# patflick/psac

Hardware: AMD Instinct MI355X
Metric: MChars/s SA+LCP build; rank-pair radix-sort HBM GB/s vs peak (higher is better)
Workload: dtype u64

## Files before the change

psac_amd/csrc/engine.hpp:

```cpp
#pragma once
#include <hip/hip_runtime.h>

#include <algorithm>
#include <cstdio>
#include <cstdlib>
#include <cstring>
#include <condition_variable>
#include <functional>
#include <map>
#include <mutex>
#include <string>
#include <thread>
#include <sched.h>
#include <pthread.h>
#include <cctype>
#include <cstdio>
#include <vector>

#include "../../include/psacx.h"
#include "radix.hpp"
#include "sa_kernels.hpp"

namespace psacx {

// ... 802 lines not shown
        } else {
            ProfScope ps(c, TC_SORT_SCATTER);
            if (small_desc) dispatch_scatter<T, uint32_t>(c, kd_in, ko_in, v_in, kd_out, ko_out, v_out, n, plan.shift[p], base, desc, sc.d_err, spec, spec_n);
            else dispatch_scatter<T, uint64_t>(c, kd_in, ko_in, v_in, kd_out, ko_out, v_out, n, plan.shift[p], base, desc, sc.d_err, spec, spec_n);
            PSACX_HIP(c, hipGetLastError());
        }
        const int form = !in.k2 ? 2 : (three ? 1 : 0);
        c->stats.scatter_launches[form] += 1;
        c->stats.scatter_records[form] += n;
        if (narrow) c->stats.scatter_bytes[form] += ((in.k2 ? 4ull : 2ull) * sizeof(T) + (v_in ? ((first && !v32_in) ? sizeof(T) : 4ull) : 0ull) + (last ? sizeof(T) : 4ull) + (dig_next ? 1ull : 0ull)) * n;
        else c->stats.scatter_bytes[form] += ((in.k2 ? 6ull : 4ull) - (v_in ? 0ull : 1ull)) * sizeof(T) * n;
        std::swap(cur, oth);
        cur.v = v_out;
    }
    if (n_exec == 0) {
        T* dst = final_v ? final_v : cur.v;
        if (iota) {
            hipLaunchKernelGGL((iota_kernel<T>), dim3(grid_for(c, n, 256)), dim3(256), 0, c->stream, dst, n, spec, spec_n);
            PSACX_HIP(c, hipGetLastError());
        } else if (v32_in && keep_v32) {
            dst = cur.v;
        } else if (v32_in) {
            T* const w = (dst == cur.v) ? oth.v : dst;
            hipLaunchKernelGGL((widen32_kernel<T>), dim3(grid_for(c, n, 256)), dim3(256), 0, c->stream, reinterpret_cast<const uint32_t*>(cur.v), n, w);
            PSACX_HIP(c, hipGetLastError());
            if (w != dst) PSACX_HIP(c, hipMemcpyAsync(dst, w, n * sizeof(T), hipMemcpyDeviceToDevice, c->stream));
        } else if (dst != cur.v) {
            PSACX_HIP(c, hipMemcpyAsync(dst, cur.v, n * sizeof(T), hipMemcpyDeviceToDevice, c->stream));
        }
        cur.v = dst;
    }
    *res = cur;
    return PSACX_OK;
}

constexpr int PSACX_RETRY_1W = 1001;
constexpr int PSACX_RETRY_1STAGE = 1002;
#ifndef PSACX_1W_ITEMS
#define PSACX_1W_ITEMS 8
#endif
inline int onew_bucket_passes(psacx_ctx* c, char* scratch, const unsigned long long* h_tabs, const OneWordLayout& lay, uint64_t* cur, uint64_t* oth, uint64_t* sa_out,
                              unsigned sfield, unsigned low, unsigned lo1, uint64_t nrec, uint64_t** s1, OneWordView* view_out = nullptr, uint8_t* dig = nullptr,
                              uint64_t in_pad = 0, uint8_t* tie_bytes = nullptr, unsigned long long* h_word = nullptr, bool* tie_bits = nullptr) {
    constexpr int BLOCK = 512, ITEMS_B = PSACX_1W_ITEMS, TILE = BLOCK * ITEMS_B;
    unsigned* tile_hist = reinterpret_cast<unsigned*>(scratch + lay.tile_hist);
    unsigned long long* slab_tot = reinterpret_cast<unsigned long long*>(scratch + lay.slab_tot);
    unsigned long long* base2 = reinterpret_cast<unsigned long long*>(scratch + lay.base2);
    unsigned long long* d_tabs = reinterpret_cast<unsigned long long*>(scratch + lay.tabs);
    OneWordTabs tb;
    tb.bucket_off = d_tabs; tb.slab_start = d_tabs + RADIX + 1; tb.slab = lay.slab;
    SlabInfo* slab_info = reinterpret_cast<SlabInfo*>(scratch + lay.slab_info);
    tb.slab_info = slab_info;
    *s1 = cur;
    if (tie_bits) *tie_bits = false;
    if (view_out) { view_out->off = d_tabs; view_out->low = low; view_out->sfield = sfield; view_out->lo1 = lo1; }
    PSACX_HIP(c, hipMemcpyAsync(d_tabs, h_tabs, 2 * (RADIX + 1) * sizeof(unsigned long long), hipMemcpyHostToDevice, c->stream));
    if (lay.total_slabs == 0) return PSACX_OK;
    const uint64_t total_slabs = lay.total_slabs, vtiles = lay.vtiles;
    hipLaunchKernelGGL(radix_slab_info_kernel<0>, dim3((unsigned)((total_slabs + 255) / 256)), dim3(256), 0, c->stream, tb.bucket_off, tb.slab_start,
                       (unsigned)total_slabs, (unsigned)(lay.slab * TILE), slab_info);
    PSACX_HIP(c, hipGetLastError());
    const int npass = (int)((low + RADIX_BITS - 1) / RADIX_BITS);
    bool first = true;
    auto tables = [&](const OneWordTabs& t, int shift, bool from_bytes, unsigned long long* dbase) {
        ProfScope ps(c, TC_SORT_TILEHIST);
        const uint64_t nt = t.tile_sub ? lay.sub_tiles : vtiles;
        if (from_bytes) hipLaunchKernelGGL((radix_tile_hist_bytes_kernel<BLOCK, ITEMS_B>), dim3((unsigned)((nt + BLOCK / WAVE - 1) / (BLOCK / WAVE))), dim3(BLOCK), 0, c->stream,
                                           (const uint8_t*)dig, t, (unsigned)nt, tile_hist);
        else
        hipLaunchKernelGGL((radix_tile_hist1w_kernel<BLOCK, ITEMS_B>), dim3((unsigned)nt), dim3(BLOCK), 0, c->stream, (const uint64_t*)cur, t, shift, tile_hist,
                           first ? in_pad : (uint64_t)0);
        if (t.tile_sub) hipLaunchKernelGGL(radix_sub_scan1w_kernel<0>, dim3(ONEW_SUB), dim3(RADIX), 0, c->stream, tile_hist, t, dbase);
        else {
            hipLaunchKernelGGL(radix_slab_scan1w_kernel<0>, dim3((unsigned)total_slabs), dim3(RADIX), 0, c->stream, tile_hist, t, (unsigned)TILE, slab_tot);
            hipLaunchKernelGGL(radix_top_scan1w_kernel<0>, dim3(RADIX), dim3(RADIX), 0, c->stream, slab_tot, t, dbase);
        }
    };
    auto scatter = [&](const OneWordTabs& t, int shift, bool widen, const unsigned long long* dbase, uint8_t* dnext, int dnext_shift) -> int {
        ProfScope ps(c, TC_SORT_SCATTER2);
        const uint64_t nt = t.tile_sub ? lay.sub_tiles : vtiles;
        PSACX_HIP(c, hipMemsetAsync(scratch, 0, 256, c->stream));
        if (!widen)
            hipLaunchKernelGGL((radix_scatter1w_kernel<BLOCK, ITEMS_B, 8>), dim3((unsigned)nt), dim3(BLOCK), 0, c->stream, (const uint64_t*)cur, oth, (uint64_t*)nullptr, shift,
                               t, dbase, tile_hist, slab_tot, reinterpret_cast<unsigned*>(scratch), sort_chunk_for(nrec, true), 0u,
                               dnext, dnext_shift, first ? in_pad : (uint64_t)0);
        else
            hipLaunchKernelGGL((radix_scatter1w_kernel<BLOCK, ITEMS_B, 9>), dim3((unsigned)nt), dim3(BLOCK), 0, c->stream, (const uint64_t*)cur, oth, sa_out, shift,
                               t, dbase, tile_hist, slab_tot, reinterpret_cast<unsigned*>(scratch), sort_chunk_for(nrec, true), lo1 | (low << 8) | (sfield << 16),
                               (uint8_t*)nullptr, 0, first ? in_pad : (uint64_t)0);
        PSACX_HIP(c, hipGetLastError());
        c->stats.scatter_launches[2] += 1; c->stats.scatter_records[2] += nrec; c->stats.scatter_bytes[2] += ((widen ? 24ull : 16ull) + (dnext ? 1ull : 0ull)) * nrec;
        c->stats.onew_passes += 1;
        std::swap(cur, oth);
        first = false;
        return PSACX_OK;
    };
    auto lsd = [&](const OneWordTabs& t, int nd, unsigned long long* dbase) -> int {
        for (int j = 0; j < nd; ++j) {
            const bool last = j + 1 == nd, widen = last && !view_out;
            const int shift = (int)sfield + j * RADIX_BITS;
            tables(t, shift, dig && j > 0, dbase);
            PSACX_HIP(c, hipGetLastError());
            PSACX_TRY(scatter(t, shift, widen, dbase, widen ? (uint8_t*)nullptr : last ? tie_bytes : dig, last ? (int)sfield : shift + RADIX_BITS));
        }
        return PSACX_OK;
    };
    if (!(lay.group && view_out && dig && tie_bytes && h_word)) {
        PSACX_TRY(lsd(tb, npass, base2));
        *s1 = cur;
        return PSACX_OK;
    }
    unsigned long long* const max_word = reinterpret_cast<unsigned long long*>(scratch + lay.max_word);
    const int mid_shift = (int)sfield + 2 * RADIX_BITS;
    OneWordTabs tg = tb;
    unsigned long long* gbase = base2;
    uint64_t ngroups = (uint64_t)RADIX * RADIX;
    if (low == 32) {
        unsigned long long* const sub_off = reinterpret_cast<unsigned long long*>(scratch + lay.sub_off);
        unsigned long long* const zero_row = reinterpret_cast<unsigned long long*>(scratch + lay.zero_row);
        unsigned* const first_tile = reinterpret_cast<unsigned*>(scratch + lay.first_tile);
        unsigned* const tile_sub = reinterpret_cast<unsigned*>(scratch + lay.tile_sub);
        tables(tb, mid_shift + RADIX_BITS, false, sub_off);
        PSACX_HIP(c, hipGetLastError());
        PSACX_TRY(scatter(tb, mid_shift + RADIX_BITS, false, sub_off, dig, mid_shift));
        {
            ProfScope ps(c, TC_SORT_TILEHIST);
            PSACX_HIP(c, hipMemcpyAsync(sub_off + ONEW_SUB, h_tabs + RADIX, sizeof(unsigned long long), hipMemcpyHostToDevice, c->stream));
            PSACX_HIP(c, hipMemsetAsync(zero_row, 0, (size_t)RADIX * 8, c->stream));
            PSACX_HIP(c, hipMemsetAsync(tile_sub, 0xFF, (size_t)lay.sub_tiles * 4, c->stream));
            hipLaunchKernelGGL(onew_sub_first_tile_kernel<1024>, dim3(1), dim3(1024), 0, c->stream, sub_off, ONEW_SUB, (unsigned)TILE, first_tile);
            hipLaunchKernelGGL(onew_sub_tile_fill_kernel<256>, dim3(ONEW_SUB / (256 / WAVE)), dim3(256), 0, c->stream, first_tile, ONEW_SUB, (unsigned)lay.sub_tiles, tile_sub);
            PSACX_HIP(c, hipGetLastError());
        }
        tg.bucket_off = sub_off; tg.tile_sub = tile_sub; tg.first_tile = first_tile; tg.zero_row = zero_row;
        gbase = reinterpret_cast<unsigned long long*>(scratch + lay.group_base);
        ngroups = (uint64_t)ONEW_SUB * RADIX;
        tables(tg, mid_shift, true, gbase);
    } else
        tables(tb, mid_shift, false, gbase);
    PSACX_HIP(c, hipMemsetAsync(max_word, 0, 16, c->stream));
    hipLaunchKernelGGL(onew_max_group_kernel<256>, dim3((unsigned)grid_for(c, ngroups, 256, 8)), dim3(256), 0, c->stream, gbase, ngroups, nrec, max_word);
    PSACX_HIP(c, hipGetLastError());
    PSACX_HIP(c, hipMemcpyAsync(h_word, max_word, sizeof(unsigned long long), hipMemcpyDeviceToHost, c->stream));
    PSACX_HIP(c, hipStreamSynchronize(c->stream));
    if (*h_word > (unsigned long long)GROUP_CAP) {
        c->stats.group_sort = 2;
        PSACX_TRY(lsd(tg, 3, gbase));
        *s1 = cur;
        return PSACX_OK;
    }
    PSACX_TRY(scatter(tg, mid_shift, false, gbase, (uint8_t*)nullptr, 0));
    {
        ProfScope ps(c, TC_SORT_SCATTER2);
        const dim3 grid((unsigned)grid_for(c, ngroups, 256, 5));
        const bool bits = tie_bits && !c->knobs.plain_side_kernels && !c->knobs.tie_bytes;
        if (bits) PSACX_HIP(c, hipMemsetAsync(tie_bytes, 0, (size_t)((nrec + 63) / 64) * 8, c->stream));
        if (bits && c->knobs.group_counting_rounds)
            hipLaunchKernelGGL((group_sort16_kernel<256, false, true>), grid, dim3(256), 0, c->stream, cur, gbase, ngroups, nrec, (int)sfield, tie_bytes);
        else if (bits)
            hipLaunchKernelGGL((group_sort16_kernel<256, true, true>), grid, dim3(256), 0, c->stream, cur, gbase, ngroups, nrec, (int)sfield, tie_bytes);
        else if (c->knobs.group_counting_rounds)
            hipLaunchKernelGGL((group_sort16_kernel<256, false>), grid, dim3(256), 0, c->stream, cur, gbase, ngroups, nrec, (int)sfield, tie_bytes);
        else
            hipLaunchKernelGGL((group_sort16_kernel<256, true>), grid, dim3(256), 0, c->stream, cur, gbase, ngroups, nrec, (int)sfield, tie_bytes);
        PSACX_HIP(c, hipGetLastError());
        if (bits) *tie_bits = true;
        c->stats.scatter_launches[2] += 1; c->stats.scatter_records[2] += nrec; c->stats.scatter_bytes[2] += 17ull * nrec;
        c->stats.onew_passes += 1;
    }
    c->stats.group_sort = 1;
    *s1 = cur;
    return PSACX_OK;
}
inline int prefix_sort_1w(psacx_ctx* c, SortScratch& sc, uint64_t* k0, uint64_t* a, uint64_t* sa_out, uint64_t n, unsigned lo1, unsigned lead,
                          psacx_round* rs, uint64_t** s1, const uint8_t* text, uint64_t n_text, const CodeTable& tab, const KeyShape& ks, bool probe,
                          OneWordView* view_out = nullptr, uint8_t* dig = nullptr, uint64_t pad = 0, uint8_t* tie_bytes = nullptr, bool* tie_bits = nullptr) {
    constexpr int BLOCK = 512, ITEMS = 8, TILE0 = BLOCK * ITEMS;
    constexpr int TILE = BLOCK * PSACX_1W_ITEMS;
    const unsigned low = lead - RADIX_BITS;
    const unsigned sfield = 64 - low;
    const uint64_t ntiles = (n + TILE0 - 1) / TILE0;
    char* const scratch = sc.d_desc;
    const PassScratch p0 = pass_scratch(scratch, ntiles);
    unsigned long long* base0 = sc.d_base;
    {
        ProfScope ps(c, TC_KMER);
        const uint64_t stride = std::max<uint64_t>(64, n >> 20), samples = n / stride;
        uint64_t slots = 1; while (slots < 4 * samples) slots <<= 1;
        unsigned long long* table = reinterpret_cast<unsigned long long*>(scratch + 256);
        unsigned long long* d_dups = reinterpret_cast<unsigned long long*>(scratch + 128);
        if (256 + slots * 8 <= sc.desc_bytes && samples >= 1024 && probe) {
            PSACX_HIP(c, hipMemsetAsync(scratch, 0, 256 + slots * 8, c->stream));
            hipLaunchKernelGGL((prefix_dup_probe_kernel<uint64_t>), dim3((unsigned)((samples + 255) / 256)), dim3(256), 0, c->stream, text, n_text, tab, ks, lo1,
                               stride, samples, table, slots, d_dups);
            PSACX_HIP(c, hipGetLastError());
            PSACX_HIP(c, hipMemcpyAsync(sc.h_base, d_dups, sizeof(unsigned long long), hipMemcpyDeviceToHost, c->stream));
            PSACX_HIP(c, hipStreamSynchronize(c->stream));
            if (sc.h_base[0] * 4 >= samples * 3) return PSACX_RETRY_1STAGE;
            if (sc.h_base[0] * 8 > samples) return PSACX_RETRY_1W;
        }
        static_assert(TILE0 == 64 * WAVE, "top_digit_hist_waves_kernel: a wave takes a tile of 64 records per lane");
        if (c->knobs.plain_side_kernels || (reinterpret_cast<uintptr_t>(p0.tile_hist) & 15u))
            hipLaunchKernelGGL((top_digit_hist_kernel<uint64_t, BLOCK, ITEMS>), dim3((unsigned)ntiles), dim3(BLOCK), 0, c->stream, text, n, n_text, tab, ks, p0.tile_hist);
        else
            hipLaunchKernelGGL((top_digit_hist_waves_kernel<256>), dim3((unsigned)grid_for(c, ntiles * WAVE, 256, 5)), dim3(256), 0, c->stream, text, n, n_text, tab, ks,
                               ntiles, p0.tile_hist);
        PSACX_HIP(c, hipGetLastError());
    }
    {
        ProfScope ps(c, TC_SORT_TILEHIST);
        launch_pass_scans(c, p0, base0);
        PSACX_HIP(c, hipGetLastError());
    }
    PSACX_HIP(c, hipMemcpyAsync(sc.h_base, base0, RADIX * sizeof(unsigned long long), hipMemcpyDeviceToHost, c->stream));
    PSACX_HIP(c, hipStreamSynchronize(c->stream));
    unsigned long long* h_tabs = sc.h_base + (PIN_TABS - PIN_BASE) / sizeof(unsigned long long);
    for (int d = 0; d < RADIX; ++d) h_tabs[d] = sc.h_base[d];
    h_tabs[RADIX] = n;
    OneWordLayout lay = onew_layout<TILE>(h_tabs, ntiles);
    if (lay.need > sc.desc_bytes || lay.vtiles >= (1ull << 31)) return PSACX_RETRY_1W;
    if (view_out && dig && tie_bytes && !c->knobs.lsd_bucket_passes) lay = onew_group_layout<TILE>(lay, n, low, sc.desc_bytes);
    unsigned long long* const h_word = sc.h_base + (PIN_GROUP_WORD - PIN_BASE) / sizeof(unsigned long long);
    {
        ProfScope ps(c, TC_KMER);
        PSACX_HIP(c, hipMemsetAsync(scratch, 0, 256, c->stream));
        hipLaunchKernelGGL((key_scatter1w_kernel<BLOCK, ITEMS>), dim3((unsigned)ntiles), dim3(BLOCK), 0, c->stream, text, n, n_text, tab, ks, pad ? k0 : a, (int)(lo1 + low),
                           base0, p0.tile_hist, p0.slab_tot, p0.counter, sort_chunk_for(n, true), p0.slab_tiles, lo1 | (sfield << 16), (uint64_t)0,
                           (uint8_t*)nullptr, 0, pad);
        PSACX_HIP(c, hipGetLastError());
    }
    uint64_t* cur = nullptr;
    if (pad) PSACX_TRY(onew_bucket_passes(c, scratch, h_tabs, lay, k0, a, sa_out, sfield, low, lo1, n, &cur, view_out, dig, pad, tie_bytes, h_word, tie_bits));
    else PSACX_TRY(onew_bucket_passes(c, scratch, h_tabs, lay, a, k0, sa_out, sfield, low, lo1, n, &cur, view_out, dig, 0, tie_bytes, h_word, tie_bits));
    *s1 = cur;
    if (rs) { rs->sort_passes = (uint32_t)((low + RADIX_BITS - 1) / RADIX_BITS + 1); rs->sort_passes_skipped = 0; }
    return PSACX_OK;
}

}
```

psac_amd/csrc/radix.hpp:

```cpp
#pragma once
#include <type_traits>
#include "dev_common.hpp"
#include "sort_scratch.hpp"
#include "group_rank.hpp"
#include "tie_bits.hpp"

namespace psacx {


struct PassPlan {
    int n_pass;
    int word[MAX_PASSES];
    int shift[MAX_PASSES];
};

inline PassPlan make_plan(int bits1, int bits2, int lo1 = 0) {
    PassPlan p;
    p.n_pass = 0;
    for (int w = 1; w >= 0; --w) {
        const int lo = w ? 0 : lo1;
        const int per = ((w ? bits2 : bits1) - lo + RADIX_BITS - 1) / RADIX_BITS;
        for (int i = 0; i < per; ++i) { p.word[p.n_pass] = w; p.shift[p.n_pass] = lo + i * RADIX_BITS; p.n_pass++; }
    }
    return p;
}

__device__ __forceinline__ void wave_hist_add(unsigned* hist, unsigned d, bool valid) {
    const uint64_t vm = __ballot(valid);
    if (vm == 0) return;
    const int first = __builtin_ctzll(vm);
    const unsigned dv = (unsigned)__builtin_amdgcn_readlane((int)d, first);
    if (__ballot(valid && d != dv) == 0) {
        if ((int)lane_id() == first) atomicAdd(&hist[dv], (unsigned)__builtin_popcountll(vm));
    } else if (valid) {
        atomicAdd(&hist[d], 1u);
    }
}

struct HistArgs {
    int n_pass;
    int word[MAX_PASSES];
    int shift[MAX_PASSES];
};

template <typename T, int BLOCK>
__global__ __launch_bounds__(BLOCK) void radix_hist_kernel(const T* __restrict__ k1,
                                                           const T* __restrict__ k2, uint64_t n,
                                                           HistArgs a,
                                                           unsigned long long* __restrict__ hist) {
    constexpr int PER = 16 / sizeof(T);
    __shared__ unsigned lh[MAX_PASSES * RADIX];
    for (int i = threadIdx.x; i < a.n_pass * RADIX; i += BLOCK) lh[i] = 0;
    __syncthreads();
    const uint64_t stride = (uint64_t)gridDim.x * BLOCK * PER;
    for (uint64_t e0 = ((uint64_t)blockIdx.x * BLOCK + threadIdx.x) * PER; e0 < n; e0 += stride) {
        T x1[PER], x2[PER];
        load_run<T, PER>(k1, e0, n, x1, (T)0);
        load_run<T, PER>(k2, e0, n, x2, (T)0);
#pragma unroll
        for (int j = 0; j < PER; ++j) {
            const bool in = e0 + j < n;
            for (int p = 0; p < a.n_pass; ++p) {
                const T w = a.word[p] ? x2[j] : x1[j];
                const unsigned d = (unsigned)(w >> a.shift[p]) & (RADIX - 1);
                wave_hist_add(&lh[p * RADIX], d, in);
            }
        }
    }
    __syncthreads();
    for (int i = threadIdx.x; i < a.n_pass * RADIX; i += BLOCK) {
        const unsigned c = lh[i];
        if (c) atomicAdd(&hist[i], (unsigned long long)c);
    }
}

template <int DUMMY>
__global__ __launch_bounds__(RADIX) void radix_hist_scan_kernel(const unsigned long long* __restrict__ hist,
                                                                 unsigned long long* __restrict__ base,
                                                                 unsigned long long n, unsigned* __restrict__ constant) {
    __shared__ unsigned long long tmp[RADIX / WAVE + 1];
    const unsigned long long h = hist[(size_t)blockIdx.x * RADIX + threadIdx.x];
    unsigned long long tot;
    const unsigned long long ex = block_scan_exclusive<RADIX, unsigned long long>(h, OpSum(), 0ull, tmp, &tot);
    base[(size_t)blockIdx.x * RADIX + threadIdx.x] = ex;
    const bool all = __syncthreads_or(h == n);
    if (threadIdx.x == 0) constant[blockIdx.x] = all ? 1u : 0u;
}

__device__ __forceinline__ uint64_t match_any8(unsigned d, bool valid) {
    uint32_t lo = 0, hi = 0;
#pragma unroll
    for (int b = 0; b < RADIX_BITS; ++b) {
        int x = __builtin_amdgcn_sbfe((int)d, (unsigned)b, 1u);
        asm("" : "+v"(x));
        const uint64_t bal = __ballot(x != 0);
        lo = __builtin_amdgcn_bitop3_b32(lo, (uint32_t)bal, (uint32_t)x, 0xF6);
        hi = __builtin_amdgcn_bitop3_b32(hi, (uint32_t)(bal >> 32), (uint32_t)x, 0xF6);
    }
    return ~(((uint64_t)hi << 32) | lo) & __ballot(valid);
}

template <typename T, int TILE, int NW> struct ScatterShared {
    T stage[TILE];
    uint8_t sdig[TILE];
    unsigned wcnt[NW * RADIX];
    unsigned bstart[RADIX];
    T goff[RADIX];
    unsigned scan_tmp[NW + 1];
    unsigned s_tile;
};

template <typename T, typename D, int BLOCK, int ITEMS, bool FULL, bool LB, bool EXT = false, bool NOKO = false, int VN = 0, int CLSB = sizeof(T), bool DNEXT3 = false>
__device__ __forceinline__ void radix_scatter_tile(
    ScatterShared<T, BLOCK * ITEMS, BLOCK / WAVE>& sh, const unsigned tile, const unsigned count,
    const T* __restrict__ kd_in, const T* __restrict__ ko_in, const T* __restrict__ v_in,
    T* __restrict__ kd_out, T* __restrict__ ko_out, T* __restrict__ v_out, int shift,
    const unsigned long long* __restrict__ digit_base, D* __restrict__ desc, unsigned* __restrict__ err,
    unsigned long long* __restrict__ dbg, const uint64_t spec, const uint64_t spec_n,
    const unsigned* __restrict__ tile_excl, const unsigned long long* __restrict__ slab_excl,
    const T* __restrict__ dsrc = nullptr, const unsigned slab_tiles = SLAB_TILES, const uint64_t voff = 0, const unsigned pack = 0,
    const T (*kd_made)[ITEMS] = nullptr, uint8_t* __restrict__ dnext = nullptr, const int dnext_shift = 0, const uint64_t out_pad = 0,
    const int dnext_ko = 0) {
    constexpr int TILE = BLOCK * ITEMS;
    constexpr int NW = BLOCK / WAVE;
    constexpr bool ONEW_IN = VN == 8 || VN == 9;
    constexpr bool ONEW_OUT = VN == 7 || VN == 8 || VN == 10;
    constexpr bool ONEW_MAKE = VN == 7 || VN == 10;
    const unsigned sfield = (ONEW_MAKE || VN == 9) ? (((pack >> 16) & 255u) ? ((pack >> 16) & 255u) : 32u) : 0u;
    T* const stage = sh.stage;
    uint8_t* const sdig = sh.sdig;
    unsigned* const wcnt = sh.wcnt;
    unsigned* const bstart = sh.bstart;
    T* const goff = sh.goff;
    unsigned* const scan_tmp = sh.scan_tmp;

    const unsigned tid = threadIdx.x;
    const unsigned lane = lane_id();
    const unsigned wave = tid / WAVE;
    const bool stamp = dbg != nullptr && (tile & 63u) == 0 && tid == 0;
    unsigned long long* mydbg = dbg + (size_t)(tile >> 6) * 8;
    if (stamp) mydbg[0] = __builtin_amdgcn_s_memtime();
    const uint64_t base = (uint64_t)tile * TILE;

    const T* __restrict__ pkd = kd_in + base;
    const T* __restrict__ pko = ko_in + base;
    const T* __restrict__ pv = v_in ? v_in + base : nullptr;
    constexpr bool LATE_EXCL = NOKO && VN != 0;
    uint64_t pre_excl = 0;
    if (!LATE_EXCL && !LB && tid < RADIX)
        pre_excl = (uint64_t)tile_excl[(uint64_t)tile * RADIX + tid] + (uint64_t)slab_excl[(uint64_t)(tile / slab_tiles) * RADIX + tid] +
                   (uint64_t)digit_base[tid];
    typedef typename std::conditional<(VN != 0) && sizeof(T) == 8, uint32_t, T>::type PV;
    T kd[ITEMS], ko[NOKO ? 1 : ITEMS];
    PV vv[ITEMS];
    unsigned char cls[EXT ? ITEMS : 1];
    const unsigned wbase = wave * (WAVE * ITEMS) + lane;
    if (EXT) {
// ... 605 lines not shown
    if (remain >= (uint64_t)TILE)
        radix_scatter_tile<uint64_t, unsigned, BLOCK, ITEMS, true, false, false, true, VN>(sh, t, (unsigned)TILE, in + off, nullptr, nullptr, out, nullptr, v_out,
                                                                                          shift, db, nullptr, nullptr, nullptr, 0, 0, te, se, nullptr, si.slab_tiles,
                                                                                          (uint64_t)b, pack, nullptr, dnext, dnext_shift);
    else
        radix_scatter_tile<uint64_t, unsigned, BLOCK, ITEMS, false, false, false, true, VN>(sh, t, (unsigned)remain, in + off, nullptr, nullptr, out, nullptr, v_out,
                                                                                           shift, db, nullptr, nullptr, nullptr, 0, 0, te, se, nullptr, si.slab_tiles,
                                                                                           (uint64_t)b, pack, nullptr, dnext, dnext_shift);
}

template <int BLOCK>
__global__ __launch_bounds__(BLOCK) void onew_sub_first_tile_kernel(const unsigned long long* __restrict__ off, unsigned nb, unsigned tile_records,
                                                                    unsigned* __restrict__ first_tile) {
    __shared__ unsigned tmp[BLOCK / WAVE + 1];
    const unsigned per = (nb + BLOCK - 1) / BLOCK, s0 = threadIdx.x * per, s1 = s0 + per < nb ? s0 + per : nb;
    unsigned sum = 0;
    for (unsigned s = s0; s < s1; ++s) sum += (unsigned)((off[s + 1] - off[s] + tile_records - 1) / tile_records);
    unsigned total;
    unsigned run = block_scan_exclusive<BLOCK, unsigned>(sum, OpSum(), 0u, tmp, &total);
    for (unsigned s = s0; s < s1; ++s) {
        first_tile[s] = run;
        run += (unsigned)((off[s + 1] - off[s] + tile_records - 1) / tile_records);
    }
    if (threadIdx.x == 0) first_tile[nb] = total;
}
template <int BLOCK>
__global__ __launch_bounds__(BLOCK) void onew_sub_tile_fill_kernel(const unsigned* __restrict__ first_tile, unsigned nb, unsigned cap, unsigned* __restrict__ tile_sub) {
    const unsigned s = blockIdx.x * (BLOCK / WAVE) + threadIdx.x / WAVE;
    if (s >= nb) return;
    const unsigned t1 = first_tile[s + 1] < cap ? first_tile[s + 1] : cap;
    for (unsigned t = first_tile[s] + lane_id(); t < t1; t += WAVE) tile_sub[t] = s;
}
template <int TAG>
__global__ __launch_bounds__(RADIX) void radix_sub_scan1w_kernel(unsigned* __restrict__ tile_hist, OneWordTabs tb, unsigned long long* __restrict__ digit_base) {
    __shared__ unsigned long long tmp[RADIX / WAVE + 1];
    const unsigned s = blockIdx.x, d = threadIdx.x;
    const unsigned t0 = tb.first_tile[s], nt = tb.first_tile[s + 1] - t0;
    unsigned* __restrict__ rows = tile_hist + (uint64_t)t0 * RADIX;
    unsigned long long run = 0;
    constexpr int B = 16;
    for (unsigned b0 = 0; b0 < nt; b0 += B) {
        unsigned v[B];
#pragma unroll
        for (int j = 0; j < B; ++j) v[j] = b0 + j < nt ? rows[(uint64_t)(b0 + j) * RADIX + d] : 0u;
#pragma unroll
        for (int j = 0; j < B; ++j) {
            if (b0 + j < nt) rows[(uint64_t)(b0 + j) * RADIX + d] = (unsigned)run;
            run += v[j];
        }
    }
    unsigned long long total;
    const unsigned long long start = block_scan_exclusive<RADIX, unsigned long long>(run, OpSum(), 0ull, tmp, &total);
    digit_base[(uint64_t)s * RADIX + d] = tb.bucket_off[s] + start;
}
template <int BLOCK>
__global__ __launch_bounds__(BLOCK) void onew_max_group_kernel(const unsigned long long* __restrict__ starts, uint64_t ngroups, uint64_t nrec,
                                                               unsigned long long* __restrict__ out) {
    unsigned long long m = 0;
    for (uint64_t g = (uint64_t)blockIdx.x * BLOCK + threadIdx.x; g < ngroups; g += (uint64_t)gridDim.x * BLOCK) {
        const unsigned long long a = starts[g], b = g + 1 < ngroups ? starts[g + 1] : (unsigned long long)nrec;
        const unsigned long long sz = b >= a ? b - a : ~0ull;
        m = sz > m ? sz : m;
    }
    m = wave_reduce<uint64_t>((uint64_t)m, OpMax());
    if (lane_id() == 0 && m) atomicMax(out, m);
}

__device__ __forceinline__ uint64_t wave_uniform64(uint64_t v) {
    const unsigned hi = (unsigned)__builtin_amdgcn_readfirstlane((int)(v >> 32)), lo = (unsigned)__builtin_amdgcn_readfirstlane((int)(unsigned)v);
    return (uint64_t)hi << 32 | lo;
}
template <int NR>
__device__ __forceinline__ bool group_rank_rows(uint64_t (&r)[GROUP_CAP / WAVE], unsigned* cnt, uint64_t* stage, const unsigned count, const int sfield,
                                                const unsigned first, const unsigned gbits, const unsigned lane) {
    static_assert(GROUP_CAP == 1 << GROUP_RANK_PLACE_BITS && GROUP_RANK_MAX + 2 <= (unsigned)WAVE, "the keys of a batch and their filler lie in half of the stage");
    unsigned* const keys = reinterpret_cast<unsigned*>(stage);
    const bool last = (unsigned)((NR - 1) * WAVE) + lane < count;
#pragma unroll
    for (int i = 0; i < RADIX / WAVE; ++i) cnt[i * WAVE + lane] = 0;
    xrun_order();
    unsigned key[NR], pos[NR], top = 0;
#pragma unroll
    for (int i = 0; i < NR; ++i) {
        const unsigned ck = group_rank_ckey(r[i], sfield, first, gbits);
        key[i] = group_rank_key(ck, (unsigned)(i * WAVE) + lane);
        pos[i] = 0;
        if (i + 1 < NR || last) pos[i] = __hip_atomic_fetch_add(&cnt[group_rank_bucket(ck, gbits)], 1u, __ATOMIC_RELAXED, __HIP_MEMORY_SCOPE_WAVEFRONT);
    }
#pragma unroll
    for (int i = 0; i < NR; ++i) top = pos[i] > top ? pos[i] : top;
    if (__ballot(!group_rank_fits(top + 1))) return false;
    xrun_order();
    {
        uint4 c4 = reinterpret_cast<uint4*>(cnt)[lane];
        const unsigned sum = c4.x + c4.y + c4.z + c4.w;
        unsigned ex = wave_scan_inclusive<unsigned>(sum, OpSum()) - sum;
        uint4 e4;
        e4.x = ex; ex += c4.x; e4.y = ex; ex += c4.y; e4.z = ex; ex += c4.z; e4.w = ex;
        reinterpret_cast<uint4*>(cnt)[lane] = e4;
    }
    xrun_order();
#pragma unroll
    for (int i = 0; i < NR; ++i) {
        const unsigned start = cnt[key[i] >> (GROUP_RANK_PLACE_BITS + 8 + gbits)];
        if (i + 1 < NR || last) keys[start + pos[i]] = key[i];
        pos[i] = i + 1 < NR || last ? start : 0u;
    }
    if (lane < GROUP_RANK_MAX + 2) keys[count + lane] = GROUP_RANK_FILL;
    xrun_order();
    unsigned below[NR];
#pragma unroll
    for (int i = 0; i < NR; ++i) below[i] = 0;
#pragma unroll
    for (unsigned j = 0; j < GROUP_RANK_MAX; j += 2) {
        if (!__ballot(j <= top)) break;
        unsigned k0[NR], k1[NR];
#pragma unroll
        for (int i = 0; i < NR; ++i) { k0[i] = keys[pos[i] + j]; k1[i] = keys[pos[i] + j + 1]; }
#pragma unroll
        for (int i = 0; i < NR; ++i) {
            below[i] += k0[i] < key[i] ? 1u : 0u; below[i] += k1[i] < key[i] ? 1u : 0u;
            asm("" : "+v"(below[i]));
        }
    }
    xrun_order();
#pragma unroll
    for (int i = 0; i < NR; ++i)
        if (i + 1 < NR || last) stage[pos[i] + below[i]] = r[i];
    xrun_order();
#pragma unroll
    for (int i = 0; i < NR; ++i)
        if (i + 1 < NR || last) r[i] = stage[(unsigned)(i * WAVE) + lane];
    xrun_order();
    return true;
}

__device__ __forceinline__ unsigned lane_before_rotating(unsigned v) {
    return (unsigned)__builtin_amdgcn_update_dpp(0, (int)v, 0x13C , 0xF, 0xF, false);
}
template <int LANE>
__device__ __forceinline__ void set_lane_at(unsigned& v, unsigned value) { asm("v_writelane_b32 %0, %1, %2" : "+v"(v) : "s"(value), "n"(LANE)); }
__device__ __forceinline__ void set_lane(unsigned& v, unsigned value, int lane) {
    switch (lane) {
    case 0: set_lane_at<0>(v, value); break;
    case 1: set_lane_at<1>(v, value); break;
    case 2: set_lane_at<2>(v, value); break;
    case 3: set_lane_at<3>(v, value); break;
    case 4: set_lane_at<4>(v, value); break;
    case 5: set_lane_at<5>(v, value); break;
    case 6: set_lane_at<6>(v, value); break;
    default: set_lane_at<7>(v, value); break;
    }
}
template <int BLOCK, bool RANK = true, bool BITS = false>
__global__ __launch_bounds__(BLOCK, RANK ? 5 : 1) void group_sort16_kernel(uint64_t* __restrict__ recs, const unsigned long long* __restrict__ starts, uint64_t ngroups,
                                                             uint64_t nrec, int sfield, uint8_t* __restrict__ tie_bytes) {
    constexpr int NW = BLOCK / WAVE, ROWS = GROUP_CAP / WAVE;
    static_assert(ROWS == 8, "set_lane: the words of a batch in the lanes 0 .. 8");
    constexpr unsigned BATCH = RANK ? GROUP_RANK_BATCH : (unsigned)GROUP_CAP;
    static_assert(GROUP_RANK_BATCH == 6 * WAVE, "group_rank_rows is instantiated for one to six rows");
    __shared__ unsigned s_cnt[NW][RADIX];
    __shared__ uint64_t s_stage[NW][GROUP_CAP];
    const unsigned wave = threadIdx.x / WAVE, lane = lane_id();
    unsigned* const cnt = s_cnt[wave];
    uint64_t* const stage = s_stage[wave];
    const uint64_t nchunks = (ngroups + WAVE - 1) / WAVE;
    for (uint64_t ch = (uint64_t)blockIdx.x * NW + wave; ch < nchunks; ch += (uint64_t)gridDim.x * NW) {
        const uint64_t g0 = ch * WAVE;
        const uint64_t s = g0 + lane < ngroups ? (uint64_t)starts[g0 + lane] : nrec;
        uint64_t snext = shfl<uint64_t>(s, (int)((lane + 1) & (WAVE - 1)));
        if (lane == WAVE - 1) snext = g0 + WAVE < ngroups ? (uint64_t)starts[g0 + WAVE] : nrec;
        if (__ballot(snext < s || snext > nrec)) continue;
        unsigned g = 0;
        while (g < (unsigned)WAVE) {
            uint64_t a = shfl<uint64_t>(s, (int)g);
            if constexpr (RANK) a = wave_uniform64(a);
            const uint64_t fit = __ballot(snext - a <= (uint64_t)BATCH) >> g;
            unsigned run = ~fit ? (unsigned)__builtin_ctzll(~fit) : (unsigned)WAVE;
            if (RANK && run == 0 && ((__ballot(snext - a <= (uint64_t)GROUP_CAP) >> g) & 1)) run = 1;
            if (run == 0) { ++g; continue; }
            unsigned count = (unsigned)(shfl<uint64_t>(snext, (int)(g + run - 1)) - a);
            if constexpr (RANK) count = __builtin_amdgcn_readfirstlane(count);
            const unsigned filled = (unsigned)__builtin_popcountll(__ballot(lane >= g && lane < g + run && snext != s));
            g += run;
            if (count == 0) continue;
            int rounds = count == 1 ? 0 : filled > 1 ? 3 : 2;
            const unsigned rows = (count + WAVE - 1) / WAVE;
            uint64_t r[ROWS];
#pragma unroll
            for (int i = 0; i < ROWS; ++i) r[i] = (unsigned)(i * WAVE) + lane < count ? recs[a + (unsigned)(i * WAVE) + lane] : 0ull;
            if (RANK && rounds) {
                const unsigned first = (unsigned)(g0 + g - run) & (RADIX - 1), gbits = group_rank_gbits(run);
                bool done = false;
                switch (__builtin_amdgcn_readfirstlane(rows)) {
                case 1: done = group_rank_rows<1>(r, cnt, stage, count, sfield, first, gbits, lane); break;
                case 2: done = group_rank_rows<2>(r, cnt, stage, count, sfield, first, gbits, lane); break;
                case 3: done = group_rank_rows<3>(r, cnt, stage, count, sfield, first, gbits, lane); break;
                case 4: done = group_rank_rows<4>(r, cnt, stage, count, sfield, first, gbits, lane); break;
                case 5: done = group_rank_rows<5>(r, cnt, stage, count, sfield, first, gbits, lane); break;
                case 6: done = group_rank_rows<6>(r, cnt, stage, count, sfield, first, gbits, lane); break;
                default: break;
                }
                if (done) rounds = 0;
            }
            for (int rd = 0; rd < rounds; ++rd) {
                const int shift = sfield + rd * RADIX_BITS;
#pragma unroll
                for (int i = 0; i < RADIX / WAVE; ++i) cnt[i * WAVE + lane] = 0;
                xrun_order();
                unsigned rank[ROWS];
#pragma unroll
                for (int i = 0; i < ROWS; ++i) {
                    if ((unsigned)i < rows) {
                        const bool valid = (unsigned)(i * WAVE) + lane < count;
                        const unsigned d = (unsigned)(r[i] >> shift) & (RADIX - 1);
                        const uint64_t m = match_any8(d, valid);
                        const unsigned prior = __hip_atomic_load(&cnt[d], __ATOMIC_RELAXED, __HIP_MEMORY_SCOPE_WAVEFRONT);
                        const unsigned below = __builtin_amdgcn_mbcnt_hi((unsigned)(m >> 32), __builtin_amdgcn_mbcnt_lo((unsigned)m, 0u));
                        if (valid && below == 0)
                            __hip_atomic_fetch_add(&cnt[d], (unsigned)__builtin_popcountll(m), __ATOMIC_RELAXED, __HIP_MEMORY_SCOPE_WAVEFRONT);
                        rank[i] = prior + below;
                    }
                }
                xrun_order();
                {
                    uint4 c4 = reinterpret_cast<uint4*>(cnt)[lane];
                    const unsigned sum = c4.x + c4.y + c4.z + c4.w;
                    unsigned ex = wave_scan_inclusive<unsigned>(sum, OpSum()) - sum;
                    uint4 e4;
                    e4.x = ex; ex += c4.x; e4.y = ex; ex += c4.y; e4.z = ex; ex += c4.z; e4.w = ex;
                    reinterpret_cast<uint4*>(cnt)[lane] = e4;
                }
                xrun_order();
#pragma unroll
                for (int i = 0; i < ROWS; ++i)
                    if ((unsigned)i < rows && (unsigned)(i * WAVE) + lane < count) stage[cnt[(unsigned)(r[i] >> shift) & (RADIX - 1)] + rank[i]] = r[i];
                xrun_order();
#pragma unroll
                for (int i = 0; i < ROWS; ++i)
                    if ((unsigned)i < rows && (unsigned)(i * WAVE) + lane < count) r[i] = stage[(unsigned)(i * WAVE) + lane];
                xrun_order();
            }
            unsigned long long mine = 0;
            uint64_t word0 = 0;
            if constexpr (BITS) {
                const uint64_t first = wave_uniform64(a);
                const unsigned ucount = (unsigned)__builtin_amdgcn_readfirstlane((int)count), urows = (unsigned)__builtin_amdgcn_readfirstlane((int)rows);
                unsigned tl = lane;
                asm volatile("" : "+v"(tl));
                unsigned mine_lo = 0, mine_hi = 0;
                uint64_t carry = 0;
                const unsigned below = 1u << (sfield - 32);
                const unsigned sh = (unsigned)first & 63u, tail = ucount & 63u;
                const uint64_t last_row = tail ? (1ull << tail) - 1ull : ~0ull;
#pragma unroll
                for (int i = 0; i < ROWS; ++i) {
                    if ((unsigned)i < urows) {
                        const unsigned hi = (unsigned)(r[i] >> 32);
                        const unsigned turn = i > 0 && tl == (unsigned)(WAVE - 1) ? (unsigned)(r[i > 0 ? i - 1 : 0] >> 32) : hi;
                        uint64_t row = __ballot((lane_before_rotating(turn) ^ hi) < below);
                        if ((unsigned)i + 1 == urows) row &= last_row;
                        if (i == 0) row &= ~1ull;
                        const uint64_t word = carry | row << sh;
                        carry = row >> 1 >> (63u - sh);
                        set_lane(mine_lo, (unsigned)word, i);
                        set_lane(mine_hi, (unsigned)(word >> 32), i);
                    }
                }
                if (tl == urows) { mine_lo = (unsigned)carry; mine_hi = (unsigned)(carry >> 32); }
                mine = (unsigned long long)mine_hi << 32 | mine_lo;
                word0 = (first >> 6) + tl;
            }
#pragma unroll
            for (int i = 0; i < ROWS; ++i)
                if ((unsigned)(i * WAVE) + lane < count) {
                    recs[a + (unsigned)(i * WAVE) + lane] = r[i];
                    if constexpr (!BITS) tie_bytes[a + (unsigned)(i * WAVE) + lane] = (uint8_t)(r[i] >> sfield);
                }
            if constexpr (BITS) if (mine) atomicOr(reinterpret_cast<unsigned long long*>(tie_bytes) + word0, mine);
        }
    }
}

}
```

Measured before the change: 31340.

## Software-pipeline group batch loads in group_sort16 kernel with lookahead prefetch

Restructures the group_sort16 kernel loop into a batch walker that prefetches the next batch's records and the next chunk's group starts while the current batch is being ranked and written back. This hides global load latency behind compute. It doubles the record registers (r and rn), so launch-bounds occupancy drops from 5 to 4 blocks and the grid size is adjusted to match. It also makes the wave index uniform via readfirstlane.

```diff
diff --git a/psac_amd/csrc/engine.hpp b/psac_amd/csrc/engine.hpp
--- a/psac_amd/csrc/engine.hpp
+++ b/psac_amd/csrc/engine.hpp
@@ -978,7 +978,7 @@
     PSACX_TRY(scatter(tg, mid_shift, false, gbase, (uint8_t*)nullptr, 0));
     {
         ProfScope ps(c, TC_SORT_SCATTER2);
-        const dim3 grid((unsigned)grid_for(c, ngroups, 256, 5));
+        const dim3 grid((unsigned)grid_for(c, ngroups, 256, 4));
         const bool bits = tie_bits && !c->knobs.plain_side_kernels && !c->knobs.tie_bytes;
         if (bits) PSACX_HIP(c, hipMemsetAsync(tie_bytes, 0, (size_t)((nrec + 63) / 64) * 8, c->stream));
         if (bits && c->knobs.group_counting_rounds)
diff --git a/psac_amd/csrc/group_batches.hpp b/psac_amd/csrc/group_batches.hpp
--- /dev/null
+++ b/psac_amd/csrc/group_batches.hpp
@@ -0,0 +1,115 @@
+#pragma once
+#include <cstdint>
+
+#if defined(__HIPCC__)
+#define PSACX_BATCH_FN __host__ __device__ __forceinline__
+#else
+#define PSACX_BATCH_FN inline
+#endif
+
+namespace psacx {
+
+constexpr unsigned GROUP_CHUNK = 64;
+
+struct GroupBatch { uint64_t group, a; unsigned run, count, filled; };
+
+PSACX_BATCH_FN uint64_t group_batch_first_chunk(unsigned workgroup, unsigned wave, unsigned waves) { return (uint64_t)workgroup * waves + wave; }
+PSACX_BATCH_FN uint64_t group_batch_chunk_stride(unsigned workgroups, unsigned waves) { return (uint64_t)workgroups * waves; }
+
+template <class Chunk>
+PSACX_BATCH_FN bool group_batch_next(const Chunk& c, uint64_t ch, unsigned& g, unsigned batch_cap, unsigned cap, bool single, GroupBatch& b) {
+    while (g < GROUP_CHUNK) {
+        const uint64_t a = c.start(g);
+        const uint64_t fit = c.ends_within(a, batch_cap) >> g;
+        unsigned run = ~fit ? (unsigned)__builtin_ctzll(~fit) : GROUP_CHUNK;
+        if (single && run == 0 && ((c.ends_within(a, cap) >> g) & 1)) run = 1;
+        if (run == 0) { ++g; continue; }
+        const unsigned count = (unsigned)(c.end(g + run - 1) - a);
+        const uint64_t in_run = (run < GROUP_CHUNK ? (1ull << run) - 1ull : ~0ull) << g;
+        const unsigned first = g;
+        g += run;
+        if (count == 0) continue;
+        b.group = ch * GROUP_CHUNK + first; b.a = a; b.run = run; b.count = count;
+        b.filled = (unsigned)__builtin_popcountll(c.nonempty() & in_run);
+        return true;
+    }
+    return false;
+}
+
+template <class Chunks>
+struct GroupBatchWalk {
+    typedef typename Chunks::Asked Asked;
+    Chunks& src;
+    typename Chunks::Chunk c;
+    uint64_t ch, stride, nchunks, nrec;
+    unsigned g, batch_cap, cap;
+    bool single, live, due, asked;
+
+    PSACX_BATCH_FN GroupBatchWalk(Chunks& src_, Asked& p, uint64_t first, uint64_t stride_, uint64_t nchunks_, uint64_t nrec_, unsigned batch_cap_, unsigned cap_,
+                                  bool single_)
+        : src(src_), c(), ch(first), stride(stride_), nchunks(nchunks_), nrec(nrec_), g(0), batch_cap(batch_cap_), cap(cap_), single(single_), live(false), due(false),
+          asked(false) {
+        if (ch < nchunks) { src.ask(ch, p); src.keep(p); enter(); }
+    }
+    PSACX_BATCH_FN void enter() {
+        c = src.take(ch);
+        live = c.valid(nrec);
+        g = 0;
+        due = stride < nchunks - ch;
+    }
+    PSACX_BATCH_FN void ask_ahead(Asked& p) {
+        if (due) { src.ask(ch + stride, p); due = false; asked = true; }
+    }
+    PSACX_BATCH_FN void arrived(const Asked& p) {
+        if (asked) { src.keep(p); asked = false; }
+    }
+    PSACX_BATCH_FN bool next(GroupBatch& b) {
+        if (ch >= nchunks) return false;
+        if (live && group_batch_next(c, ch, g, batch_cap, cap, single, b)) return true;
+        while (stride < nchunks - ch) {
+            if (due) { Asked p; src.ask(ch + stride, p); src.keep(p); }
+            ch += stride;
+            enter();
+            if (live && group_batch_next(c, ch, g, batch_cap, cap, single, b)) return true;
+        }
+        ch = nchunks;
+        return false;
+    }
+};
+
+struct GroupChunkHost {
+    uint64_t s[GROUP_CHUNK + 1];
+    uint64_t start(unsigned l) const { return s[l]; }
+    uint64_t end(unsigned l) const { return s[l + 1]; }
+    uint64_t ends_within(uint64_t a, uint64_t cap) const {
+        uint64_t m = 0;
+        for (unsigned l = 0; l < GROUP_CHUNK; ++l) m |= (uint64_t)(s[l + 1] - a <= cap) << l;
+        return m;
+    }
+    uint64_t nonempty() const {
+        uint64_t m = 0;
+        for (unsigned l = 0; l < GROUP_CHUNK; ++l) m |= (uint64_t)(s[l + 1] != s[l]) << l;
+        return m;
+    }
+    bool valid(uint64_t nrec) const {
+        bool good = true;
+        for (unsigned l = 0; l < GROUP_CHUNK; ++l) good = good && s[l + 1] >= s[l] && s[l + 1] <= nrec;
+        return good;
+    }
+};
+struct GroupChunksHost {
+    typedef GroupChunkHost Chunk;
+    typedef uint64_t Asked;
+    const uint64_t* starts;
+    uint64_t ngroups, nrec, kept;
+    void ask(uint64_t ch, Asked& p) { p = ch; }
+    void keep(const Asked& p) { kept = p; }
+    Chunk take(uint64_t ch) const {
+        Chunk c;
+        for (unsigned l = 0; l <= GROUP_CHUNK; ++l) c.s[l] = ch * GROUP_CHUNK + l < ngroups ? starts[ch * GROUP_CHUNK + l] : nrec;
+        if (kept != ch) c.s[0] = nrec + 1;
+        return c;
+    }
+};
+
+}
diff --git a/psac_amd/csrc/radix.hpp b/psac_amd/csrc/radix.hpp
--- a/psac_amd/csrc/radix.hpp
+++ b/psac_amd/csrc/radix.hpp
@@ -3,6 +3,7 @@
 #include "dev_common.hpp"
 #include "sort_scratch.hpp"
 #include "group_rank.hpp"
+#include "group_batches.hpp"
 #include "tie_bits.hpp"
 
 namespace psacx {
@@ -914,45 +915,78 @@
     default: set_lane_at<7>(v, value); break;
     }
 }
+template <bool UNIFORM>
+struct GroupChunkWave {
+    uint64_t s, snext;
+    __device__ __forceinline__ uint64_t start(unsigned l) const { const uint64_t v = shfl<uint64_t>(s, (int)l); return UNIFORM ? wave_uniform64(v) : v; }
+    __device__ __forceinline__ uint64_t end(unsigned l) const { const uint64_t v = shfl<uint64_t>(snext, (int)l); return UNIFORM ? wave_uniform64(v) : v; }
+    __device__ __forceinline__ uint64_t ends_within(uint64_t a, uint64_t cap) const { return __ballot(snext - a <= cap); }
+    __device__ __forceinline__ uint64_t nonempty() const { return __ballot(snext != s); }
+    __device__ __forceinline__ bool valid(uint64_t nrec) const { return !__ballot(snext < s || snext > nrec); }
+};
+struct GroupStartsAsked { uint64_t s, e; };
+template <bool UNIFORM>
+struct GroupChunksWave {
+    typedef GroupChunkWave<UNIFORM> Chunk;
+    typedef GroupStartsAsked Asked;
+    const unsigned long long* __restrict__ starts;
+    uint64_t ngroups, nrec;
+    unsigned lane;
+    uint64_t s, e;
+    __device__ __forceinline__ void ask(uint64_t ch, Asked& p) const {
+        const uint64_t g0 = ch * WAVE;
+        p.s = g0 + lane < ngroups ? (uint64_t)starts[g0 + lane] : nrec;
+        p.e = nrec;
+        if (lane == WAVE - 1) p.e = g0 + WAVE < ngroups ? (uint64_t)starts[g0 + WAVE] : nrec;
+    }
+    __device__ __forceinline__ void keep(const Asked& p) { s = p.s; e = p.e; }
+    __device__ __forceinline__ Chunk take(uint64_t) const {
+        Chunk c;
+        c.s = s;
+        c.snext = shfl<uint64_t>(s, (int)((lane + 1) & (WAVE - 1)));
+        if (lane == WAVE - 1) c.snext = e;
+        return c;
+    }
+};
 template <int BLOCK, bool RANK = true, bool BITS = false>
-__global__ __launch_bounds__(BLOCK, RANK ? 5 : 1) void group_sort16_kernel(uint64_t* __restrict__ recs, const unsigned long long* __restrict__ starts, uint64_t ngroups,
+__global__ __launch_bounds__(BLOCK, RANK ? 4 : 1) void group_sort16_kernel(uint64_t* __restrict__ recs, const unsigned long long* __restrict__ starts, uint64_t ngroups,
                                                              uint64_t nrec, int sfield, uint8_t* __restrict__ tie_bytes) {
     constexpr int NW = BLOCK / WAVE, ROWS = GROUP_CAP / WAVE;
     static_assert(ROWS == 8, "set_lane: the words of a batch in the lanes 0 .. 8");
+    static_assert(GROUP_CHUNK == (unsigned)WAVE, "a chunk of the walk is a group per lane");
     constexpr unsigned BATCH = RANK ? GROUP_RANK_BATCH : (unsigned)GROUP_CAP;
     static_assert(GROUP_RANK_BATCH == 6 * WAVE, "group_rank_rows is instantiated for one to six rows");
     __shared__ unsigned s_cnt[NW][RADIX];
     __shared__ uint64_t s_stage[NW][GROUP_CAP];
-    const unsigned wave = threadIdx.x / WAVE, lane = lane_id();
+    const unsigned wave = (unsigned)__builtin_amdgcn_readfirstlane((int)(threadIdx.x / WAVE)), lane = lane_id();
     unsigned* const cnt = s_cnt[wave];
     uint64_t* const stage = s_stage[wave];
     const uint64_t nchunks = (ngroups + WAVE - 1) / WAVE;
-    for (uint64_t ch = (uint64_t)blockIdx.x * NW + wave; ch < nchunks; ch += (uint64_t)gridDim.x * NW) {
-        const uint64_t g0 = ch * WAVE;
-        const uint64_t s = g0 + lane < ngroups ? (uint64_t)starts[g0 + lane] : nrec;
-        uint64_t snext = shfl<uint64_t>(s, (int)((lane + 1) & (WAVE - 1)));
-        if (lane == WAVE - 1) snext = g0 + WAVE < ngroups ? (uint64_t)starts[g0 + WAVE] : nrec;
-        if (__ballot(snext < s || snext > nrec)) continue;
-        unsigned g = 0;
-        while (g < (unsigned)WAVE) {
-            uint64_t a = shfl<uint64_t>(s, (int)g);
-            if constexpr (RANK) a = wave_uniform64(a);
-            const uint64_t fit = __ballot(snext - a <= (uint64_t)BATCH) >> g;
-            unsigned run = ~fit ? (unsigned)__builtin_ctzll(~fit) : (unsigned)WAVE;
-            if (RANK && run == 0 && ((__ballot(snext - a <= (uint64_t)GROUP_CAP) >> g) & 1)) run = 1;
-            if (run == 0) { ++g; continue; }
-            unsigned count = (unsigned)(shfl<uint64_t>(snext, (int)(g + run - 1)) - a);
-            if constexpr (RANK) count = __builtin_amdgcn_readfirstlane(count);
-            const unsigned filled = (unsigned)__builtin_popcountll(__ballot(lane >= g && lane < g + run && snext != s));
-            g += run;
-            if (count == 0) continue;
-            int rounds = count == 1 ? 0 : filled > 1 ? 3 : 2;
+    GroupChunksWave<RANK> chunks{starts, ngroups, nrec, lane, 0, 0};
+    GroupStartsAsked asked_first;
+    GroupBatchWalk<GroupChunksWave<RANK>> walk(chunks, asked_first, group_batch_first_chunk(blockIdx.x, wave, NW), group_batch_chunk_stride(gridDim.x, NW), nchunks, nrec,
+                                               BATCH, (unsigned)GROUP_CAP, RANK);
+    GroupBatch b, ahead;
+    if (walk.next(b)) {
+        walk.ask_ahead(asked_first);
+        uint64_t r[ROWS], rn[ROWS];
+#pragma unroll
+        for (int i = 0; i < ROWS; ++i) r[i] = (unsigned)(i * WAVE) + lane < b.count ? recs[b.a + (unsigned)(i * WAVE) + lane] : 0ull;
+#pragma unroll
+        for (int i = 0; i < ROWS; ++i) asm volatile("" : "+v"(r[i]));
+        walk.arrived(asked_first);
+        for (bool more = true; more;) {
+            GroupStartsAsked asked;
+            more = walk.next(ahead);
+            walk.ask_ahead(asked);
+#pragma unroll
+            for (int i = 0; i < ROWS; ++i) rn[i] = more && (unsigned)(i * WAVE) + lane < ahead.count ? recs[ahead.a + (unsigned)(i * WAVE) + lane] : 0ull;
+            const uint64_t a = b.a;
+            const unsigned count = b.count, run = b.run;
+            int rounds = count == 1 ? 0 : b.filled > 1 ? 3 : 2;
             const unsigned rows = (count + WAVE - 1) / WAVE;
-            uint64_t r[ROWS];
-#pragma unroll
-            for (int i = 0; i < ROWS; ++i) r[i] = (unsigned)(i * WAVE) + lane < count ? recs[a + (unsigned)(i * WAVE) + lane] : 0ull;
             if (RANK && rounds) {
-                const unsigned first = (unsigned)(g0 + g - run) & (RADIX - 1), gbits = group_rank_gbits(run);
+                const unsigned first = (unsigned)b.group & (RADIX - 1), gbits = group_rank_gbits(run);
                 bool done = false;
                 switch (__builtin_amdgcn_readfirstlane(rows)) {
                 case 1: done = group_rank_rows<1>(r, cnt, stage, count, sfield, first, gbits, lane); break;
@@ -1034,14 +1068,20 @@
                 word0 = (first >> 6) + tl;
             }
 #pragma unroll
+            for (int i = 0; i < ROWS; ++i) asm volatile("" : "+v"(rn[i]));
+            walk.arrived(asked);
+#pragma unroll
             for (int i = 0; i < ROWS; ++i)
                 if ((unsigned)(i * WAVE) + lane < count) {
                     recs[a + (unsigned)(i * WAVE) + lane] = r[i];
                     if constexpr (!BITS) tie_bytes[a + (unsigned)(i * WAVE) + lane] = (uint8_t)(r[i] >> sfield);
                 }
             if constexpr (BITS) if (mine) atomicOr(reinterpret_cast<unsigned long long*>(tie_bytes) + word0, mine);
-        }
-    }
-}
-
-}
+#pragma unroll
+            for (int i = 0; i < ROWS; ++i) r[i] = rn[i];
+            b = ahead;
+        }
+    }
+}
+
+}
```

Result: no change. 31270 (-0.2%).
